# abeauvisage/uasl_motion_estimation

Hardware: AMD Instinct MI355X
Metric: frames/sec + BA iter/sec, 2000 feats x 20-keyframe window, 1/2/4/8 MI355X (higher is better)
Workload: dtype u8+f32 (MI), f64 (BA); 1 GPU; config 3: 1280x720 stereo, 2000 feats, 20-keyframe window, 11x11 MI patches; frame=KLT + MI scale LM (LM, MAX_NB_ITER 10, tolerances off) + 10 BA LM iterations, parallelism=1 independent streams (one per GPU)

## Files before the change

### uasl_motion_estimation_amd/csrc/api.hip

```cpp
#include <vector>
#include "me_internal.hpp"
#include <algorithm>
#include <cstring>
#include <rocprofiler-sdk-roctx/roctx.h>

me_range::me_range(const char* name) { roctxRangePushA(name); }
me_range::~me_range() { roctxRangePop(); }

typedef float me_f4v __attribute__((ext_vector_type(4)));
__global__ __launch_bounds__(256) void copy_f4_kernel(const me_f4v* __restrict__ a, me_f4v* __restrict__ b, size_t n) {
  const size_t stride = (size_t)gridDim.x * 256;
  for (size_t i = (size_t)blockIdx.x * 256 + threadIdx.x; i < n; i += stride)
    __builtin_nontemporal_store(__builtin_nontemporal_load(&a[i]), &b[i]);
}

static int hbm_copy_gbs(me_ctx* c, size_t bytes, int reps, double* gbs) {
  void *a = nullptr, *b = nullptr;
  ME_HIP(c, hipMalloc(&a, bytes));
  hipError_t e = hipMalloc(&b, bytes);
  if (e != hipSuccess) {
    (void)hipFree(a);
    return me_set_error(c, ME_ERR_NOMEM, "me_hbm_copy_gbs: hipMalloc(%zu) failed", bytes);
  }
  const size_t n = bytes / 16;
// ... 16 lines not shown
  if (e0) (void)hipEventDestroy(e0);
  if (e1) (void)hipEventDestroy(e1);
  (void)hipFree(a);
  (void)hipFree(b);
  if (rc == ME_OK) *gbs = 2.0 * (double)(n * 16) * reps / (ms * 1e-3) / 1e9;
  return rc;
}

int me_set_error(me_ctx* ctx, int code, const char* fmt, ...) {
  if (ctx) {
    char buf[1024];
    va_list ap;
    va_start(ap, fmt);
    vsnprintf(buf, sizeof(buf), fmt, ap);
    va_end(ap);
    ctx->err = buf;
  }
  return code;
}

int me_scratch(me_ctx* ctx, int slot, size_t bytes, void** out) {
  if ((int)ctx->slot_ptr.size() <= slot) {
    ctx->slot_ptr.resize(slot + 1, nullptr);
    ctx->slot_size.resize(slot + 1, 0);
  }
  if (bytes == 0) bytes = 16;
  if (ctx->slot_size[slot] < bytes) {
    if (ctx->slot_ptr[slot]) {
      ME_HIP(ctx, hipStreamSynchronize(ctx->stream));
      ME_HIP(ctx, hipFree(ctx->slot_ptr[slot]));
      ctx->slot_ptr[slot] = nullptr;
      ctx->slot_size[slot] = 0;
    }
    size_t sz = bytes + bytes / 4;
    void* p = nullptr;
    hipError_t e = hipMalloc(&p, sz);
    if (e != hipSuccess) return me_set_error(ctx, ME_ERR_NOMEM, "hipMalloc(%zu) failed: %s", sz, hipGetErrorString(e));
    ctx->slot_ptr[slot] = p;
    ctx->slot_size[slot] = sz;
  }
  *out = ctx->slot_ptr[slot];
  return ME_OK;
}

int me_pinned(me_ctx* ctx, size_t bytes, void** out) {
  if (ctx->pinned_size < bytes) {
    if (ctx->pinned) {
      ME_HIP(ctx, hipStreamSynchronize(ctx->stream));
      ME_HIP(ctx, hipHostFree(ctx->pinned));
    }
    ctx->pinned = nullptr;
    ctx->pinned_size = 0;
    size_t sz = bytes < 4096 ? 4096 : bytes;
    ME_HIP(ctx, hipHostMalloc(&ctx->pinned, sz, hipHostMallocDefault));
    ctx->pinned_size = sz;
  }
  *out = ctx->pinned;
  return ME_OK;
}

int me_check_launch(me_ctx* ctx, const char* what) {
  hipError_t e = hipGetLastError();
  if (e != hipSuccess) return me_set_error(ctx, ME_ERR_HIP, "launch of %s failed: %s", what, hipGetErrorString(e));
  return ME_OK;
}

static hipEvent_t pool_get(me_ctx* c) {
  if (!c->event_pool.empty()) {
    hipEvent_t e = c->event_pool.back();
    c->event_pool.pop_back();
    return e;
  }
  hipEvent_t e = nullptr;
  if (hipEventCreate(&e) != hipSuccess) return nullptr;
  return e;
}

me_ktimer::me_ktimer(me_ctx* ctx, int kernel, bool ext_launch) : c(ctx), k(kernel), ext(ext_launch) {
  if (c && (c->timing >> kernel & 1) && c->kt_seen[kernel]++ % c->timing_every == 0) {
    a = pool_get(c);
    b = pool_get(c);
    if (!a || !b) a = b = nullptr;
    if (a && !ext) hipEventRecord(a, c->stream);
  }
}
me_ktimer::~me_ktimer() {
  if (c && a && b) {
    if (!ext) hipEventRecord(b, c->stream);
    c->pending.push_back({a, b, k});
  }
}

static void drain_timers(me_ctx* c) {
  for (auto& p : c->pending) {
    hipEventSynchronize(p.b);
    float ms = 0;
    if (hipEventElapsedTime(&ms, p.a, p.b) == hipSuccess) {
      c->launches[p.kernel] += 1;
      c->total_ms[p.kernel] += ms;
    }
    c->event_pool.push_back(p.a);
    c->event_pool.push_back(p.b);
  }
  c->pending.clear();
}

extern "C" {
// ... 184 lines not shown
```

### uasl_motion_estimation_amd/csrc/ba.hip

```cpp
#include <algorithm>
#include <cmath>
#include <cstdio>
#include <cstring>
#include <mutex>
#include <numeric>
#include <vector>
#include <hip/hip_ext.h>
#include "me_internal.hpp"
#include "ba_kernels.hpp"
#include "roster.hpp"
#include "solve_diag.hpp"
#include "me_device.hpp"

using me_dev::wave_sync;

using namespace ba;

namespace {

constexpr double kDblMin = 2.2250738585072014e-308;
constexpr double kDblEps = 2.220446049250313e-16;

template <int Ctrl>
__device__ __forceinline__ double dpp_f64(double x);
// ... 176 lines not shown
  }
  for (int k = 12; k < 24; ++k) Jc[k] = 0.0;
  for (int k = 6; k < 12; ++k) Jp[k] = 0.0;
}

template <int OD>
__device__ __forceinline__ void obs_residual(const Geo& g, const Bufs& b, long o, const double* cam, const double* X,
                                             double* r, double* Jc, double* Jp) {
  if (OD == 4)
    stereo_residual(g, cam, X, b.obs + 4 * o, r, Jc, Jp);
  else
    mono_residual(g, cam, X, b.obs + 2 * o, b.cam_id[o] != 0, r, Jc, Jp);
}

__device__ __forceinline__ void huber(double s, double* rho0, double* sqrt_rho1) {
  if (s > 1.0) {
    const double rr = sqrt(s);
    *rho0 = 2.0 * rr - 1.0;
    *sqrt_rho1 = sqrt(fmax(kDblMin, 1.0 / rr));
  } else {
    *rho0 = s;
    *sqrt_rho1 = 1.0;
  }
}

template <bool SC1>
__device__ __forceinline__ double a_ld(const double* p) {
  if (!SC1) return *p;
  return __builtin_bit_cast(double, __hip_atomic_load(reinterpret_cast<const unsigned long long*>(p), ME_HO_LD,
                                                      __HIP_MEMORY_SCOPE_AGENT));
}
template <bool SC1>
__device__ __forceinline__ void a_st(double* p, double v) {
  if (!SC1) {
    *p = v;
    return;
  }
  __hip_atomic_store(reinterpret_cast<unsigned long long*>(p), __builtin_bit_cast(unsigned long long, v),
                     ME_HO_ST, __HIP_MEMORY_SCOPE_AGENT);
}
__device__ __forceinline__ void drain_and_barrier() {
  asm volatile("s_waitcnt vmcnt(0)" ::: "memory");
  __syncthreads();
}


constexpr int kPtBlock = 64;

#ifndef ME_LIN_SMALL
#define ME_LIN_SMALL 64
#endif
constexpr int kLinSmall = ME_LIN_SMALL, kLinSmallMaxObs = 64 * 512;
__host__ __device__ inline int lin_block(int no) { return no <= kLinSmallMaxObs ? kLinSmall : kBlock; }
template <int OD, int BLK>
__global__ __launch_bounds__(BLK) void linearize_kernel(Geo g, Bufs b) {
  __shared__ double lds[BLK / 64];
  const State* st = b.st;
  if (st->done || !st->need_lin) return;
  const int o = blockIdx.x * BLK + threadIdx.x;
  double cost = 0;
  if (o < g.no) {
    const int cur = st->cur;
    const int ci = b.cam_idx[o], pi = b.pt_idx[o];
    double r[4], Jc[24], Jp[12];
    obs_residual<OD>(g, b, o, b.cams[cur] + 6 * ci, b.pts[cur] + 3 * pi, r, Jc, Jp);
    const double s = r[0] * r[0] + r[1] * r[1] + r[2] * r[2] + r[3] * r[3];
    double rho0, sc;
    huber(s, &rho0, &sc);
    cost = 0.5 * rho0;
    for (int k = 0; k < 4; ++k) r[k] *= sc;
    for (int k = 0; k < 24; ++k) Jc[k] *= sc;
    for (int k = 0; k < 12; ++k) Jp[k] *= sc;
    const long slot = b.pos[o];
    double* X = b.obsx + slot * kObsxStride;
    X[0] = Jp[0] * Jp[0] + Jp[3] * Jp[3] + Jp[6] * Jp[6] + Jp[9] * Jp[9];
    X[1] = Jp[0] * Jp[1] + Jp[3] * Jp[4] + Jp[6] * Jp[7] + Jp[9] * Jp[10];
    X[2] = Jp[0] * Jp[2] + Jp[3] * Jp[5] + Jp[6] * Jp[8] + Jp[9] * Jp[11];
    X[3] = Jp[1] * Jp[1] + Jp[4] * Jp[4] + Jp[7] * Jp[7] + Jp[10] * Jp[10];
    X[4] = Jp[1] * Jp[2] + Jp[4] * Jp[5] + Jp[7] * Jp[8] + Jp[10] * Jp[11];
    X[5] = Jp[2] * Jp[2] + Jp[5] * Jp[5] + Jp[8] * Jp[8] + Jp[11] * Jp[11];
    for (int a = 0; a < 3; ++a) X[6 + a] = Jp[a] * r[0] + Jp[3 + a] * r[1] + Jp[6 + a] * r[2] + Jp[9 + a] * r[3];
    if (ci - g.nf >= 0) {
      double* W = b.Wo + 18 * slot;
      for (int a = 0; a < 6; ++a)
        for (int c = 0; c < 3; ++c)
          W[a * 3 + c] = Jc[a] * Jp[c] + Jc[6 + a] * Jp[3 + c] + Jc[12 + a] * Jp[6 + c] + Jc[18 + a] * Jp[9 + c];
    }
  }
  double v[1] = {cost};
  double out[1];
  block_sum<1>(v, out, lds);
  if (threadIdx.x == 0) b.part[R_COST * g.pstride + blockIdx.x] = out[0];
}

__device__ __forceinline__ bool last_arrival_wt(unsigned* cnt, unsigned expected) {
  __shared__ int slast;
  __syncthreads();
  if (threadIdx.x == 0) {
    asm volatile("s_waitcnt vmcnt(0)" ::: "memory");
    const unsigned k = __hip_atomic_fetch_add(cnt, 1u, ME_HO_RMW, __HIP_MEMORY_SCOPE_AGENT);
    slast = k == expected - 1;
    if (slast) __hip_atomic_store(cnt, 0u, __ATOMIC_RELAXED, __HIP_MEMORY_SCOPE_AGENT);
  }
  __syncthreads();
  return slast != 0;
}

__device__ void cam_reduce_body(const Geo& g, const Bufs& b, int sharded, const double* cpart, double* colnorm,
                                double* gc_raw, double* Uraw, int ci, int first, int count) {
  __shared__ double tot[27];
  __shared__ double csl[6];
  const State* st = b.st;
  const int u = threadIdx.x;
  if (u < 27) {
    double sum = 0.0;
    for (int k = 0; k < count; ++k) sum += a_ld<true>(&cpart[27 * ((long)first + k) + u]);
    tot[u] = sum;
    if (u < 21) Uraw[21 * (long)ci + u] = sum;
    else gc_raw[6 * ci + u - 21] = sum;
  }
  __syncthreads();
  if (u < 6) {
    const int d = u * 6 - u * (u - 1) / 2;
    colnorm[6 * ci + u] = tot[d];
    if (!sharded) {
      double* cs = b.csc + 6 * ci;
      if (!st->scaled) cs[u] = g.jacobi ? 1.0 / (1.0 + sqrt(tot[d])) : 1.0;
      csl[u] = cs[u];
    }
  }
  if (sharded) return;
  __syncthreads();
  if (u < 21) {
    int a = 0, r = u;
    while (r >= 6 - a) {
      r -= 6 - a;
      ++a;
    }
    const int c = a + r;
    const double x = tot[u] * csl[a] * csl[c];
    double* U = b.U + 36 * (long)ci;
// ... 49 lines not shown
    huber(s2, &rho0, &sc);
    for (int kk = 0; kk < 4; ++kk) r[kk] *= sc;
    for (int kk = 0; kk < 24; ++kk) Jc[kk] *= sc;
    int u = 0;
    for (int a = 0; a < 6; ++a)
      for (int c = a; c < 6; ++c, ++u)
        v[u] += Jc[a] * Jc[c] + Jc[6 + a] * Jc[6 + c] + Jc[12 + a] * Jc[12 + c] + Jc[18 + a] * Jc[18 + c];
    for (int a = 0; a < 6; ++a) v[21 + a] += Jc[a] * r[0] + Jc[6 + a] * r[1] + Jc[12 + a] * r[2] + Jc[18 + a] * r[3];
  }
  CAM_T(1);
#pragma unroll
  for (int u = 0; u < 27; ++u) {
    double x = v[u];
    x += dpp_f64<kDppQuadSwap1>(x);
    x += dpp_f64<kDppQuadSwap2>(x);
    x += dpp_f64<kDppRowHalfMirror>(x);
    x += dpp_f64<kDppRowMirror>(x);
    v[u] = x;
  }
  if ((threadIdx.x & 15) == 0)
#pragma unroll
    for (int u = 0; u < 27; ++u) rows[(threadIdx.x >> 4) * 27 + u] = v[u];
  __syncthreads();
  CAM_T(2);
  if (threadIdx.x < 27) {
    double sum = 0.0;
#pragma unroll
    for (int r = 0; r < kBlock / 16; ++r) sum += rows[r * 27 + threadIdx.x];
    a_st<true>(&cpart[27 * (long)un + threadIdx.x], sum);
  }
  const bool last = last_arrival_wt(b.cnt + ci, (unsigned)ue.w);
  CAM_T(3);
  if (!last) return;
  cam_reduce_body(g, b, sharded, cpart, colnorm, gc_raw, Uraw, ci, ufirst, ue.w);
  CAM_T(4);
#ifdef ME_CAM_TS
  if (un == g_cam_ts_unit && threadIdx.x == 0) atomicAdd(&g_cam_ts[5], 1ull);
#endif
}

__global__ __launch_bounds__(kBlock) void cam_assemble_kernel(Geo g, Bufs b, double* cpart, int sharded,
                                                              double* colnorm, double* gc_raw, double* Uraw) {
  if (g.od == 4)
    cam_assemble_body<4>(g, b, cpart, sharded, colnorm, gc_raw, Uraw, blockIdx.x);
  else
    cam_assemble_body<2>(g, b, cpart, sharded, colnorm, gc_raw, Uraw, blockIdx.x);
}

struct CamArgs {
  double *cpart, *colnorm, *gc_raw, *Uraw;
  int on;
  int ncam;
};

__global__ void xch_flags_kernel(Geo g, Bufs b, double* colnorm) {
  colnorm[g.n6] = b.st->bad_input ? 1.0 : 0.0;
  colnorm[g.n6 + 1] = b.st->infeasible ? 1.0 : 0.0;
}

__global__ void cam_finish_kernel(Geo g, Bufs b, const double* colnorm, const double* gc_raw, const double* Uraw,
                                  int first) {
  State* st = b.st;
  if (first) {
    const bool bad = colnorm[g.n6] != 0.0, infeasible = colnorm[g.n6 + 1] != 0.0;
    __syncthreads();
    if (bad || infeasible) {
      if (blockIdx.x == 0 && threadIdx.x == 0) {
        st->bad_input = bad;
        st->infeasible = infeasible;
        st->done = 1;
        st->termination = 2;
      }
      return;
    }
  }
  if (st->done || !st->need_lin) return;
  const int ci = blockIdx.x * blockDim.x + threadIdx.x;
  if (ci >= g.m) return;
  double* cs = b.csc + 6 * ci;
  if (!st->scaled)
    for (int a = 0; a < 6; ++a) cs[a] = g.jacobi ? 1.0 / (1.0 + sqrt(colnorm[6 * ci + a])) : 1.0;
  const double* Ur = Uraw + 21 * (long)ci;
  double* U = b.U + 36 * (long)ci;
  int u = 0;
  for (int a = 0; a < 6; ++a)
    for (int c = a; c < 6; ++c, ++u) {
      const double x = Ur[u] * cs[a] * cs[c];
      U[a * 6 + c] = x;
      U[c * 6 + a] = x;
    }
  for (int a = 0; a < 6; ++a) b.gcs[6 * ci + a] = gc_raw[6 * ci + a] * cs[a];
}

__device__ __forceinline__ bool chol3(const double* A, double* L) {
  double d0 = A[0];
  if (!(d0 > 0)) return false;
  d0 = sqrt(d0);
  const double l10 = A[3] / d0, l20 = A[6] / d0;
  double d1 = A[4] - l10 * l10;
  if (!(d1 > 0)) return false;
  d1 = sqrt(d1);
  const double l21 = (A[7] - l20 * l10) / d1;
  double d2 = A[8] - l20 * l20 - l21 * l21;
  if (!(d2 > 0)) return false;
  d2 = sqrt(d2);
  L[0] = d0; L[1] = 0; L[2] = 0;
// ... 2171 lines not shown
  int run = wsum[wv] + x - s;
  for (long i = beg; i < end; ++i) {
    const int v = b.phist[i];
    b.phist[i] = run;
    run += v;
  }
  __syncthreads();
  for (int j = t; j < g.np; j += kScanBlock) {
    const int key = b.pkey[j];
    const int pos = b.phist[(long)key * g.nblkp + j / kBlock] + b.prank[j];
    b.order[pos] = j;
    const int r = pos / g.rlen;
    if (pos == r * g.rlen) rA[r] = key / g.T;
    atomicMax(&rB[r], key % g.T);
  }
  __syncthreads();
  for (int r = t; r < g.nruns; r += kScanBlock) {
    const int B = max(rA[r], rB[r]);
    rB[r] = B;
    b.rband[2 * r] = rA[r];
    b.rband[2 * r + 1] = B;
  }
  __syncthreads();
  for (int p = t; p < g.npairs; p += kScanBlock) {
    int I = 0, rem = p;
    while (rem >= g.T - I) {
      rem -= g.T - I;
      ++I;
    }
    const int J = I + rem;
    int cnt = 0;
    for (int r = 0; r < g.nruns; ++r) {
      const int A = rA[r], B = rB[r];
      const int nb = B - A + 1, ns = nb + (B < g.T - 1 ? 1 : 0);
      const int ka = (I >= A && I <= B) ? I - A : (I == g.T - 1 ? nb : -1);
      const int kb = (J >= A && J <= B) ? J - A : (J == g.T - 1 ? nb : -1);
      if (ka < 0 || kb < 0) continue;
      b.tl[(long)p * g.nruns + cnt++] = r * g.npairs + ka * ns - ka * (ka - 1) / 2 + (kb - ka);
    }
    b.tcnt[p] = cnt;
    for (int q = cnt; q < g.nruns; ++q) b.tl[(long)p * g.nruns + q] = -1;
  }
}

__global__ __launch_bounds__(kBlock) void output_kernel(Geo g, Bufs b, double* cams_dst, double* pts_dst) {
  const int cur = b.st->cur;
  const long gid = (long)blockIdx.x * kBlock + threadIdx.x;
  constexpr int kStateWords = (int)(sizeof(State) / 8);
  if (gid < kStateWords) b.out[gid] = ((const double*)b.st)[gid];
  if (gid < 6 * (long)g.nc) cams_dst[gid] = b.cams[cur][gid];
  if (gid < 3 * (long)g.np) pts_dst[gid] = b.pts[cur][gid];
}

struct Plan {
  me_ctx* c = nullptr;
  Geo g;
  unsigned asm_gen = 0;
  Bufs b;
  Opts o;
  double* colnorm = nullptr;
  double* gc_raw = nullptr;
  double* Uraw = nullptr;
  double* cpart = nullptr;
  double* host = nullptr;
  State* hstate[2] = {nullptr, nullptr};
  bool dev = false;
  bool copy_out = false;
  bool reserve_only = false;
  size_t solve_lds = 0;
  size_t schur_lds = 0;
  int use_lds = 0;
  int solve_flags = 0;
  int n_enq = 0;
  bool no_fused_asm = false;
  bool full_S = false;
  int solve_cap = 0;
  me_comm* comm = nullptr;
  bool xmax_separate = false;
};

inline long rup(long x, long m) { return (x + m - 1) / m * m; }
int blocks(long n, int bs) { return (int)std::max(1L, (n + bs - 1) / bs); }

void schur_geometry(int npairs, int np, int Rpad, Geo& g) {
  const bool wide = schur_lds_bytes(kSchurPtsWide, Rpad) <= kSchurLdsCap;
  const bool split_wide = wide && npairs <= 40 && np <= 256 * kSchurPts;
  g.spts = wide ? kSchurPtsWide : npairs > 100 ? kSchurPtsSmall : kSchurPts;
  g.nsub = (int)std::max(1L, ((long)np + g.spts - 1) / g.spts);
  g.rsub = (int)std::max(1L, ((long)g.nsub + 255) / 256);
  g.rlen = g.spts * g.rsub;
  g.nruns = (int)std::max(1L, ((long)np + g.rlen - 1) / g.rlen);
  const int nt = split_wide ? 2 : npairs > 100 ? kSchurNtMax : std::min(kSchurNtMax, 4);
  g.stpw = 8 * std::min((npairs + 7) / 8, nt);
  g.sgrp = (npairs + g.stpw - 1) / g.stpw;
  g.ksplit = (g.sgrp > 1 ? (int)rup((long)g.nruns, 8) : g.nruns) * g.sgrp;
  g.sorted = npairs > 40 ? 1 : 0;
}

void ba_geometry(Geo& g, int n_cams, int fixed_frames, int n_pts) {
  g.nc = n_cams;
  g.np = n_pts;
  g.nf = std::min(std::max(fixed_frames, 0), n_cams);
  g.m = g.nc - g.nf;
  g.n6 = 6 * g.m;
  g.Rpad = (int)rup(g.n6 + 1, 16);
  g.T = g.Rpad / 16;
  g.Ts = (g.n6 + 1 + 15) / 16;
  g.npairs = g.T * (g.T + 1) / 2;
  schur_geometry(g.npairs, g.np, g.Rpad, g);
}

constexpr size_t kSolveLdsCap = 150 * 1024;
inline int solve_form(int Ts) {
  if (8 * (solve_small_doubles(Ts) + solve_a_doubles(Ts)) <= kSolveLdsCap) return 0;
  return Ts >= kSolveMwMinTs ? 2 : 1;
}

extern "C" int me_debug_ba_geometry(int n_cams, int fixed_frames, int n_pts, int* out) {
  if (n_cams <= 0 || n_pts < 0 || !out) return ME_ERR_INVALID;
  Geo g;
  ba_geometry(g, n_cams, fixed_frames, n_pts);
  const int v[10] = {g.spts, g.nsub, g.rsub, g.rlen, g.nruns, g.stpw, g.sgrp, g.ksplit, g.sorted, solve_form(g.Ts)};
  std::memcpy(out, v, sizeof v);
  return ME_OK;
}

int ba_drain(me_ctx* c);

int plan_build(me_ctx* c, const me_ba_problem* p, const me_ba_options* opt, Plan& P, int slot_base,
               int async = -1, me_comm* comm = nullptr) {
  if (async < 0) ME_TRY(ba_drain(c));
  ME_CHECK(c, p->n_cams > 0 && p->n_pts >= 0 && p->n_obs >= 0, "BA: bad sizes");
  ME_CHECK(c, p->n_cams <= kMaxScanCams, "BA: at most %d cameras per window", kMaxScanCams);
  ME_CHECK(c, p->obs_dim == 0 || p->obs_dim == 2 || p->obs_dim == 4, "BA: obs_dim must be 2 or 4 (Observation<M>)");
  const bool mono = p->obs_dim == 2;
  ME_CHECK(c, p->feat_var > 0 && (mono || p->baseline != 0.0), "BA: wrong calibration parameters (BundleAdjuster.h:147)");
  ME_CHECK(c, !mono || p->cam_id || p->n_obs == 0, "BA: obs_dim 2 needs cam_id (Observation::camID)");
  const double baseline = mono && p->baseline == 0 ? 0.5 : p->baseline;
  ME_CHECK(c, p->mem == ME_HOST || p->mem == ME_DEVICE, "BA: bad memory kind");
  if (p->mem == ME_HOST) {
    for (int i = 0; i < p->n_obs; ++i) {
      ME_CHECK(c, p->cam_idx[i] >= 0 && p->cam_idx[i] < p->n_cams && p->pt_idx[i] >= 0 && p->pt_idx[i] < p->n_pts,
               "BA: observation %d indexes outside the window", i);
    }
  }
  P.c = c;
  int hook = c->dbg_solve_flags;
  if ((hook & kFlagFailEveryOther) && (c->dbg_solve_count++ & 1)) hook |= kFlagSolveFail;
  P.no_fused_asm = (hook & kFlagSeparateAsm) != 0;
  P.solve_flags = hook & (kFlagAsmTimeout | kFlagSolveFail | kFlagRosterNow);
  Geo& g = P.g;
  ba_geometry(g, p->n_cams, p->fixed_frames, p->n_pts);
  g.no = p->n_obs;
  g.od = mono ? 2 : 4;
  P.comm = comm;
  P.xmax_separate = comm && comm->world == 0;
  g.xslots = comm && comm->world > 0 ? comm->world : 1;
  g.xrank = comm && comm->world > 0 ? comm->rank : 0;
  ME_CHECK(c, g.nruns <= kMaxRuns, "BA: %d Schur runs exceed %d", g.nruns, kMaxRuns);
  g.nblkp = blocks(std::max(g.np, 1), kBlock);
  ME_CHECK(c, g.npairs <= 8 * 24, "BA: %d variable cameras exceed the Schur tile budget", g.m);
  g.nblk_obs = (int)std::max(1L, rup(std::max(g.no, 1), kBlock) / kBlock);
  g.nblk_lin = (int)std::max(1L, rup(std::max(g.no, 1), lin_block(g.no)) / lin_block(g.no));
  g.nblk_pts = (int)std::max(1L, rup(std::max(g.np, 1), kPtBlock) / kPtBlock);
  g.jacobi = opt->jacobi_scaling ? 1 : 0;
  g.ncu = (int)(rup(std::max(g.no, 1), kBlock) / kBlock) + g.m;
  g.nblk_step = (int)std::max(1L, rup(std::max(g.np, 1), kStepPts) / kStepPts);
  g.pstride = std::max({g.nblk_obs, g.nblk_lin, g.nblk_pts, g.nblk_step, g.ksplit});
  std::memcpy(g.K0, p->K0, sizeof(g.K0));
  std::memcpy(g.K1, p->K1, sizeof(g.K1));
  g.baseline = baseline;
  g.sinv = 1.0 / std::sqrt(p->feat_var);
  const double Zmax = p->K0[0] * baseline / 0.1;
  const double Zmin = p->K0[0] * baseline / (2 * p->K0[2]);
  g.hi[0] = Zmax / p->K0[0] * p->K0[2];
  g.hi[1] = Zmax / p->K0[4] * p->K0[5];
  g.hi[2] = Zmax;
  g.lo[0] = -Zmax / p->K0[0] * p->K0[2];
  g.lo[1] = -Zmax / p->K0[4] * p->K0[5];
  g.lo[2] = Zmin;
// ... 12 lines not shown
  const bool dev = p->mem == ME_DEVICE;
  const long nb = g.pstride;
  Bufs& b = P.b;
  std::vector<std::pair<size_t, void**>> items;
  auto add = [&](size_t bytes, void* dst) { items.push_back({rup((long)std::max<size_t>(bytes, 8), 256), (void**)dst}); };
  add(8 * 6 * (size_t)g.nc, &b.cams[0]);
  add(8 * 3 * (size_t)g.np, &b.pts[0]);
  add(8 * g.od * (size_t)g.no, &b.obs);
  add(4 * (size_t)g.no, &b.cam_idx);
  add(4 * (size_t)g.no, &b.pt_idx);
  add(mono ? 4 * (size_t)g.no : 0, &b.cam_id);
  const size_t n_inputs = items.size();
  add(8 * 6 * (size_t)g.nc, &b.cams[1]);
  add(8 * 3 * (size_t)g.np, &b.pts[1]);
  add(4 * (size_t)(g.np + 1), &b.p_off);
  add(4 * (size_t)g.no, &b.p_obs);
  add(4 * (size_t)g.no, &b.pos);
  add(4 * (size_t)g.no, &b.p_cam);
  add(4 * (size_t)(g.m + 1), &b.c_off);
  add(4 * (size_t)g.no, &b.c_obs);
  add(4 * (size_t)g.no, &b.tmp_obs);
  add(4 * (size_t)g.no, &b.cpos);
  add(8 * kObsxStride * (size_t)g.no, &b.obsx);
  add((size_t)g.no, &b.dup);
  add(8 * solve_a_doubles(g.Ts), &b.Abuf);
  add(8 * 18 * (size_t)g.no, &b.Wo);
  add(8 * (size_t)g.n6, &b.csc);
  add(8 * 3 * (size_t)g.np, &b.psc);
  add(8 * 36 * (size_t)g.m, &b.U);
  add(8 * (size_t)g.n6, &b.gcs);
  add(8 * 9 * (size_t)g.np, &b.V);
  add(8 * 3 * (size_t)g.np, &b.gps);
  add(8 * 9 * (size_t)g.np, &b.Lp);
  add(8 * 3 * (size_t)g.np, &b.zp);
  add(8 * 256 * (size_t)g.nruns * g.npairs, &b.Spart);
  add(4 * (size_t)std::max(g.np, 1), &b.order);
  add(4 * (size_t)std::max(g.np, 1), &b.pkey);
  add(4 * (size_t)std::max(g.np, 1), &b.prank);
  add(4 * (size_t)g.T * g.T * g.nblkp, &b.phist);
  add(8 * (size_t)g.nruns, &b.rband);
  add(4 * (size_t)g.npairs * g.nruns, &b.tl);
  add(4 * (size_t)g.npairs, &b.tcnt);
  add(8 * (size_t)g.n6 * g.n6 + 8 * (size_t)(2 * g.n6 + 2), &b.S);
  add(8 * (size_t)g.n6, &b.yc);
  add(8 * 3 * (size_t)g.np, &b.dp);
  add(8 * R_COUNT * (size_t)nb, &b.part);
  add(8 * (R_COUNT + 2), &b.scal);
  add(sizeof(State), &b.st);
  add(8 * (size_t)(g.n6 + 2), &P.colnorm);
  add(8 * (size_t)g.n6, &P.gc_raw);
  add(8 * 21 * (size_t)std::max(g.m, 1), &P.Uraw);
  add(8 * 27 * (size_t)g.ncu, &P.cpart);
  add(4 * (size_t)kCuStride * (size_t)rup(g.ncu, 8), &b.cunit);
  add(4 * (size_t)(g.m + 1 + 3 + 2), &b.cnt);
  add(4 * (size_t)blocks((long)g.npairs * 256, kSolveBlock / kSaGroups), &b.asm_claim);
  const size_t work_bytes = 4 * (2 * (size_t)g.np + (size_t)g.nblk_obs * g.nc + 4);
  add(work_bytes, &b.work);
  const size_t out_doubles = sizeof(State) / 8 + 6 * (size_t)g.nc + 3 * (size_t)g.np;
  add(8 * out_doubles, &b.out);
  b.xch = nullptr;
  if (comm) add(8 * (size_t)xo_total(g), &b.xch);
  size_t total = 0, input_span = 0;
  for (size_t k = 0; k < items.size(); ++k) {
    total += items[k].first;
    if (k < n_inputs) input_span += items[k].first;
  }
  void* arena;
  ME_TRY(me_scratch(c, SLOT_COUNT + slot_base, total, &arena));
  char* ptr = (char*)arena;
  for (auto& it : items) {
    *it.second = ptr;
    ptr += it.first;
  }
  b.ssync = b.cnt + g.m + 1;
  b.roster = b.cnt + g.m + 4;
  b.bvec = b.S + (size_t)g.n6 * g.n6;
  b.diagU = b.bvec + g.n6;
  void* hp;
  const size_t stage = rup((long)std::max(8 * out_doubles, dev ? (size_t)0 : input_span), 64);
  const size_t hbytes = stage + 2 * rup(sizeof(State), 64);
  if (async >= 0) {
    if (c->ba_pinned_size[async] < hbytes) {
      if (c->ba_pinned[async]) ME_HIP(c, hipHostFree(c->ba_pinned[async]));
      c->ba_pinned[async] = nullptr;
      c->ba_pinned_size[async] = 0;
      ME_HIP(c, hipHostMalloc(&c->ba_pinned[async], std::max(hbytes, (size_t)4096), hipHostMallocDefault));
      c->ba_pinned_size[async] = std::max(hbytes, (size_t)4096);
    }
    hp = c->ba_pinned[async];
  } else {
    ME_TRY(me_pinned(c, hbytes, &hp));
  }
  P.host = (double*)hp;
  if (P.reserve_only) return ME_OK;
  P.hstate[0] = (State*)((char*)hp + stage);
  P.hstate[1] = (State*)((char*)hp + stage + rup(sizeof(State), 64));
  P.dev = dev;
  hipStream_t s = c->stream;
  if (!dev) {
    char* h = (char*)hp;
    const void* src[6] = {p->cams, p->pts, p->obs, p->cam_idx, p->pt_idx, p->cam_id};
    const size_t len[6] = {8 * 6 * (size_t)g.nc, 8 * 3 * (size_t)g.np, 8 * g.od * (size_t)g.no, 4 * (size_t)g.no,
                           4 * (size_t)g.no, mono ? 4 * (size_t)g.no : 0};
    size_t off = 0;
    for (int k = 0; k < 6; ++k) {
      if (len[k]) std::memcpy(h + off, src[k], len[k]);
      off += items[k].first;
    }
    ME_HIP(c, hipMemcpyAsync(b.cams[0], hp, input_span, hipMemcpyHostToDevice, s));
  } else {
    b.obs = p->obs;
    b.cam_idx = p->cam_idx;
    b.pt_idx = p->pt_idx;
    if (mono) b.cam_id = p->cam_id;
  }
  ME_HIP(c, hipMemsetAsync(b.cnt, 0, (size_t)((char*)b.work - (char*)b.cnt) + work_bytes, s));
  P.asm_gen = 0;
  const double* cams_in = dev ? p->cams : b.cams[0];
  const double* pts_in = dev ? p->pts : b.pts[0];
  const long nthr = std::max({(long)g.nblk_obs * kBlock, (long)g.np, 6L * g.nc, 3L * g.np});
  hipLaunchKernelGGL(plan_count_kernel, dim3(blocks(nthr, kBlock)), dim3(kBlock), 4 * (size_t)g.nc, s, g, b, cams_in,
                     pts_in);
  hipLaunchKernelGGL(plan_scan_kernel, dim3(1), dim3(kScanBlock), 0, s, g, b, o);
  hipLaunchKernelGGL(plan_scatter_kernel, dim3(g.nblk_obs), dim3(kBlock), 0, s, g, b);
  hipLaunchKernelGGL(plan_segsort_kernel, dim3(blocks(std::max(g.np, 1), kSortBlock / 64)), dim3(kSortBlock), 0, s, g,
                     b);
  if (g.sorted) {
    hipLaunchKernelGGL(plan_band_kernel, dim3(g.nblkp), dim3(kBlock), 0, s, g, b);
    hipLaunchKernelGGL(plan_order_kernel, dim3(1), dim3(kScanBlock), 0, s, g, b);
  }
  ME_TRY(me_check_launch(c, "BA plan"));
  P.use_lds = solve_form(g.Ts) == 0 ? 1 : 0;
  P.solve_lds = 8 * (solve_small_doubles(g.Ts) + (P.use_lds ? solve_a_doubles(g.Ts) : 0));
  ME_CHECK(c, P.solve_lds <= kSolveLdsCap, "BA: %d variable cameras exceed the camera-solve workspace", g.m);
  P.schur_lds = schur_lds_bytes(g.spts, g.Rpad);
  ME_CHECK(c, P.schur_lds <= kSchurLdsCap, "BA: %d variable cameras exceed the Schur workspace", g.m);
  if (!c->ba_lds_attr) {
    for (const void* k : {(const void*)cam_solve_kernel<0>, (const void*)cam_solve_kernel<1>, (const void*)cam_solve_kernel<2>})
      ME_HIP(c, hipFuncSetAttribute(k, hipFuncAttributeMaxDynamicSharedMemorySize, (int)kSolveLdsCap));
#define ME_SCHUR_K(N)                                                                                   \
  (const void*)pt_schur_kernel<N, 512, kSchurPts>, (const void*)pt_schur_kernel<N, 512, kSchurPtsWide>, \
      (const void*)pt_schur_kernel<N, 512, kSchurPtsSmall>
    for (const void* k : {ME_SCHUR_K(2), ME_SCHUR_K(3), ME_SCHUR_K(4), ME_SCHUR_K(5)})
#undef ME_SCHUR_K
      ME_HIP(c, hipFuncSetAttribute(k, hipFuncAttributeMaxDynamicSharedMemorySize, (int)kSchurLdsCap));
    c->ba_lds_attr = 1;
  }
  if (!P.use_lds) {
    int per_cu = 0;
    ME_HIP(c, hipOccupancyMaxActiveBlocksPerMultiprocessor(&per_cu, cam_solve_kernel<2>, kSolveBlock, P.solve_lds));
    P.solve_cap = std::max(0, per_cu) * (c->cu_active > 0 ? c->cu_active : c->num_cu);
    if (P.comm && g.Ts >= kSolveMwMinTs) {
      double* d = P.b.scal;
      const double v = -(double)P.solve_cap;
      ME_HIP(c, hipMemcpyAsync(d, &v, 8, hipMemcpyHostToDevice, c->stream));
      ME_TRY(me_comm_allreduce_impl(P.comm, d, 1, ME_COMM_MAX));
      double r = 0.0;
      ME_HIP(c, hipMemcpyAsync(&r, d, 8, hipMemcpyDeviceToHost, c->stream));
      ME_HIP(c, hipStreamSynchronize(c->stream));
      P.solve_cap = (int)-r;
    }
  }
  return ME_OK;
}



#define ME_XCH(ptr, n, op) ME_TRY(me_comm_allreduce_impl(P.comm, (ptr), (long)(n), (op)))

int enqueue_linearize(Plan& P) {
  me_ctx* c = P.c;
  const Geo& g = P.g;
  hipStream_t s = c->stream;
  const bool sh = P.comm != nullptr;
  {
    me_ktimer t(c, ME_KT_BA_LINEARIZE);
    const bool small = lin_block(g.no) == kLinSmall;
    if (g.od == 4 && small)
      hipLaunchKernelGGL((linearize_kernel<4, kLinSmall>), dim3(g.nblk_lin), dim3(kLinSmall), 0, s, g, P.b);
    else if (g.od == 4)
      hipLaunchKernelGGL((linearize_kernel<4, kBlock>), dim3(g.nblk_lin), dim3(kBlock), 0, s, g, P.b);
    else if (small)
      hipLaunchKernelGGL((linearize_kernel<2, kLinSmall>), dim3(g.nblk_lin), dim3(kLinSmall), 0, s, g, P.b);
    else
      hipLaunchKernelGGL((linearize_kernel<2, kBlock>), dim3(g.nblk_lin), dim3(kBlock), 0, s, g, P.b);
  }
  const bool first = P.n_enq == 0;
  const bool fused = !first && g.m > 0;
  ++P.n_enq;
  CamArgs ca{P.cpart, P.colnorm, P.gc_raw, P.Uraw, fused ? 1 : 0, fused ? (g.ncu + 7) / 8 * 8 : 0};
  if (g.m > 0 && !fused)
    hipLaunchKernelGGL(cam_assemble_kernel, dim3(g.ncu), dim3(kBlock), 0, s, g, P.b, P.cpart, sh ? 1 : 0,
                       P.colnorm, P.gc_raw, P.Uraw);
  if (sh && !fused) {
    if (first) {
      hipLaunchKernelGGL(xch_flags_kernel, dim3(1), dim3(1), 0, s, g, P.b, P.colnorm);
      ME_XCH(P.colnorm, g.n6 + 2, ME_COMM_SUM);
    }
    hipLaunchKernelGGL(cam_finish_kernel, dim3(blocks(std::max(g.m, 1), 64)), dim3(64), 0, s, g, P.b,
                       (const double*)P.colnorm, (const double*)P.gc_raw, (const double*)P.Uraw, first ? 1 : 0);
  }
  {
    me_ktimer t(c, ME_KT_BA_SCHUR, true);
    const int pw8 = g.stpw / 8;
    const dim3 grd(g.ksplit + ca.ncam);
#define ME_SCHUR(N)                                                                                          \
  do {                                                                                                       \
    if (g.spts == kSchurPtsWide)                                                                             \
      hipExtLaunchKernelGGL((pt_schur_kernel<N, 512, kSchurPtsWide>), grd, dim3(512), P.schur_lds, s, t.a, t.b, 0, g, \
                            P.b, P.o, ca);                                                                   \
    else if (g.spts == kSchurPtsSmall)                                                                       \
      hipExtLaunchKernelGGL((pt_schur_kernel<N, 512, kSchurPtsSmall>), grd, dim3(512), P.schur_lds, s, t.a, t.b, 0, g, \
                            P.b, P.o, ca);                                                                   \
    else                                                                                                     \
      hipExtLaunchKernelGGL((pt_schur_kernel<N, 512, kSchurPts>), grd, dim3(512), P.schur_lds, s, t.a, t.b, 0, g, P.b, \
                            P.o, ca);                                                                        \
  } while (0)
    static_assert(kSchurNtMax >= 3 && kSchurNtMax <= 5, "instantiated tile counts");
    if (pw8 <= 2) ME_SCHUR(2);
    else if (pw8 <= 3) ME_SCHUR(3);
    else if (pw8 <= 4) ME_SCHUR(4);
    else ME_SCHUR(5);
#undef ME_SCHUR
  }
  if (sh) {
    hipLaunchKernelGGL(s_assemble_kernel, dim3(blocks((long)g.npairs * 256, kSaElems) + 1), dim3(kBlock), 0, s, g,
                       P.b, P.o, (const double*)P.gc_raw, 0, (int)SA_PACK);
    if (P.xmax_separate) {
      ME_XCH(P.b.xch, xo_gmax(g), ME_COMM_SUM);
      ME_XCH(P.b.xch + xo_gmax(g), 1, ME_COMM_MAX);
    } else {
      ME_XCH(P.b.xch, xo_total(g), ME_COMM_SUM);
    }
  }
  return me_check_launch(c, "BA linearize");
}

int enqueue_assemble(Plan& P, bool img = false) {
  me_ctx* c = P.c;
  const Geo& g = P.g;
  const int mode = P.comm ? SA_UNPACK : SA_SUM;
  if (g.m > 0)
    hipLaunchKernelGGL(s_assemble_kernel, dim3(blocks((long)g.npairs * 256, kSaElems) + 1), dim3(kBlock), 0,
                       c->stream, g, P.b, P.o, (const double*)P.gc_raw, P.full_S ? 1 : 0, mode,
                       img && !P.full_S ? P.b.Abuf : nullptr);
  else
    hipLaunchKernelGGL(lin_finalize_kernel, dim3(1), dim3(kFinBlock), 0, c->stream, g, P.b, P.o,
                       (const double*)P.gc_raw);
  return me_check_launch(c, "BA assemble");
}

int enqueue_iteration(Plan& P, bool last = false) {
  me_ctx* c = P.c;
  const Geo& g = P.g;
  hipStream_t s = c->stream;
  const bool sh = P.comm != nullptr;
  ME_TRY(enqueue_linearize(P));
  const int np0 = (g.Ts - 1) * g.Ts / 2;
  int nwk = solve_form(g.Ts) == 2 ? std::min(64, std::max(1, (np0 + kSolveBlock / 64 - 1) / (kSolveBlock / 64))) : 0;
  nwk = std::max(0, std::min(nwk, P.solve_cap - 1));
  const bool fuse = g.m > 0 && !P.full_S && !last && nwk == 0 && !P.no_fused_asm;
  const int nasm = fuse ? blocks((long)g.npairs * 256, kSolveBlock / kSaGroups) : 0;
  const bool img = !fuse && !last && g.m > 0 && !P.full_S && ME_SOLVE_IMG;
  if (!fuse) ME_TRY(enqueue_assemble(P, img));
  if (last) return me_check_launch(c, "BA iteration");
  if (g.m == 0) ME_HIP(c, hipMemsetAsync(P.b.scal + R_COUNT, 0, 8, s));
  {
    me_ktimer t(c, ME_KT_BA_SOLVE);
    const double* gc = P.gc_raw;
    const int sk = P.solve_flags | (img ? kFlagImg : 0);
    const unsigned gen = nasm > 0 ? ++P.asm_gen : 0u;
    if (P.use_lds)
      hipLaunchKernelGGL(cam_solve_kernel<0>, dim3(1 + nasm), dim3(kSolveBlock), P.solve_lds, s, g, P.b, P.o, sk, 0,
                         nasm, gc, gen);
    else if (nwk > 0)
#ifdef ME_COOP_LAUNCH
    {
      int skv = sk, nwv = nwk, z = 0;
      unsigned gv = gen;
      void* args[] = {(void*)&g, (void*)&P.b, (void*)&P.o, &skv, &nwv, &z, (void*)&gc, &gv};
      ME_HIP(c, hipLaunchCooperativeKernel((const void*)cam_solve_kernel<2>, dim3(1 + nwk), dim3(kSolveBlock), args,
                                           (unsigned)P.solve_lds, s));
    }
#else
      hipLaunchKernelGGL(cam_solve_kernel<2>, dim3(1 + nwk), dim3(kSolveBlock), P.solve_lds, s, g, P.b, P.o, sk, nwk,
                         0, gc, gen);
#endif
    else
      hipLaunchKernelGGL(cam_solve_kernel<1>, dim3(1 + nasm), dim3(kSolveBlock), P.solve_lds, s, g, P.b, P.o, sk, 0,
                         nasm, gc, gen);
  }
  {
    me_ktimer t(c, ME_KT_BA_STEP);
    if (g.od == 4)
      hipLaunchKernelGGL(pt_step_kernel<4>, dim3(g.nblk_step + 1), dim3(kStepBlock), 0, s, g, P.b, P.o, sh ? 0 : 1);
    else
      hipLaunchKernelGGL(pt_step_kernel<2>, dim3(g.nblk_step + 1), dim3(kStepBlock), 0, s, g, P.b, P.o, sh ? 0 : 1);
  }
  if (sh) {
    ME_XCH(P.b.scal + R_MODEL, 5, ME_COMM_SUM);
    hipLaunchKernelGGL(decide_kernel, dim3(1), dim3(64), 0, s, g, P.b, P.o);
  }
  return me_check_launch(c, "BA iteration");
}

int enqueue_output(Plan& P, me_ba_problem* p) {
  me_ctx* c = P.c;
  const Geo& g = P.g;
  constexpr size_t nst = sizeof(State) / 8;
  double* cams_dst = P.dev ? p->cams : P.b.out + nst;
  double* pts_dst = P.dev ? p->pts : P.b.out + nst + 6 * (size_t)g.nc;
  const long n = std::max({(long)nst, 6L * g.nc, 3L * g.np});
  hipLaunchKernelGGL(output_kernel, dim3(blocks(n, kBlock)), dim3(kBlock), 0, c->stream, g, P.b, cams_dst, pts_dst);
  ME_TRY(me_check_launch(c, "BA output"));
  const size_t bytes = 8 * (P.dev ? nst : nst + 6 * (size_t)g.nc + 3 * (size_t)g.np);
  ME_HIP(c, hipMemcpyAsync(P.host, P.b.out, bytes, hipMemcpyDeviceToHost, c->stream));
  if (P.dev && P.copy_out) {
    ME_HIP(c, hipMemcpyAsync(P.host + nst, p->cams, 8 * 6 * (size_t)g.nc, hipMemcpyDeviceToHost, c->stream));
    if (g.np)
      ME_HIP(c, hipMemcpyAsync(P.host + nst + 6 * (size_t)g.nc, p->pts, 8 * 3 * (size_t)g.np, hipMemcpyDeviceToHost,
                               c->stream));
  }
  return ME_OK;
}

int finish(Plan& P, me_ba_problem* p, me_ba_summary* sum, bool output_queued = false, hipEvent_t done = nullptr) {
  me_ctx* c = P.c;
  const Geo& g = P.g;
  constexpr size_t nst = sizeof(State) / 8;
  static_assert(sizeof(State) % 8 == 0, "State is read back as doubles");
  if (!output_queued) ME_TRY(enqueue_output(P, p));
  if (done) ME_HIP(c, hipEventSynchronize(done));
  else ME_HIP(c, hipStreamSynchronize(c->stream));
  State st;
  std::memcpy(&st, P.host, sizeof(State));
  std::memcpy(P.c->dbg, st.stamps, sizeof(st.stamps));
  if (!P.dev) {
    std::memcpy(p->cams, P.host + nst, 8 * 6 * (size_t)g.nc);
    if (g.np) std::memcpy(p->pts, P.host + nst + 6 * (size_t)g.nc, 8 * 3 * (size_t)g.np);
  }
  if (st.bad_input) return me_set_error(c, ME_ERR_INVALID, "BA: an observation indexes outside the window");
  if (st.spin_err)
    return me_set_error(c, ME_ERR_STATE,
                        "BA: a cross-workgroup hand-off of the camera solve timed out (workgroups not co-resident: "
                        "CU mask or concurrent persistent kernels; wait sites 0x%x: 1 worker roster, 2 worker step "
                        "poll, 4 fused assemblers, 8 LDS step flags, 16 workers' count, 32 backward flags, 0 the "
                        "step exchange)",
                        (unsigned)st.pad[0]);
  if (sum) {
    sum->termination = st.termination;
    sum->iterations = st.iterations;
    sum->successful_steps = st.successful;
    sum->initial_cost = st.initial_cost;
    sum->final_cost = st.x_cost;
    sum->status = st.termination == 2 ? 3 : 2;
    if (st.infeasible) {
      sum->iterations = 0;
      sum->successful_steps = 0;
      sum->initial_cost = sum->final_cost = NAN;
    }
  }
  return ME_OK;
}

int solve_impl(me_ctx* c, me_ba_problem* p, const me_ba_options* opt, me_comm* comm, me_ba_summary* sum) {
  me_range range_("me_ba_solve");
  if (!c || !p || !opt) return ME_ERR_INVALID;
  ME_HIP(c, hipSetDevice(c->device));
  Plan P;
  ME_TRY(plan_build(c, p, opt, P, 0, -1, comm));
  const int chunk = 4;
  int it = 0;
  auto enqueue_chunk = [&](int slot) -> int {
    for (int k = 0; k < chunk && it <= opt->max_num_iterations; ++k, ++it)
      ME_TRY(enqueue_iteration(P, it == opt->max_num_iterations));
    ME_HIP(c, hipMemcpyAsync(P.hstate[slot], P.b.st, sizeof(State), hipMemcpyDeviceToHost, c->stream));
    ME_HIP(c, hipEventRecord(c->poll_ev[slot], c->stream));
    return ME_OK;
  };
  bool out_q = false;
  ME_TRY(enqueue_chunk(0));
  if (it > opt->max_num_iterations) {
    ME_TRY(enqueue_output(P, p));
    out_q = true;
  }
  for (int cur = 0;; cur ^= 1) {
    const bool more = it <= opt->max_num_iterations;
    if (more) {
      ME_TRY(enqueue_chunk(cur ^ 1));
      if (it > opt->max_num_iterations) {
        ME_TRY(enqueue_output(P, p));
        out_q = true;
      }
    }
    ME_HIP(c, hipEventSynchronize(c->poll_ev[cur]));
    if (P.hstate[cur]->done || !more) break;
  }
  return finish(P, p, sum, out_q);
}

struct AsyncSolve {
  Plan P;
  me_ba_problem prob;
  hipEvent_t ev = nullptr;
  int set = 0;
  bool completed = false;
  int rc = ME_OK;
  me_ba_summary sum{};
};
constexpr int kBaQueue = 2;
struct AsyncQueue {
  AsyncSolve* q[kBaQueue] = {nullptr, nullptr};
  int n = 0;
  AsyncSolve* last = nullptr;
  int last_set = 1;
  std::mutex mu;
};

int ba_complete_one(me_ctx* c, AsyncSolve* A) {
  if (A->completed) return ME_OK;
  A->rc = finish(A->P, &A->prob, &A->sum, true, A->ev);
  A->completed = true;
  return ME_OK;
}

void ba_async_free(me_ctx* c) {
  auto* Q = (AsyncQueue*)c->ba_async;
  if (!Q) return;
  for (int i = 0; i < Q->n; ++i) {
    AsyncSolve* A = Q->q[i];
    if (!A->completed) hipEventSynchronize(A->ev);
    hipEventDestroy(A->ev);
    delete A;
  }
  delete Q->last;
  delete Q;
  c->ba_async = nullptr;
  c->ba_async_free = nullptr;
}

AsyncQueue* ba_queue(me_ctx* c) {
  if (!c->ba_async) {
    c->ba_async = new AsyncQueue;
    c->ba_async_free = ba_async_free;
  }
  return (AsyncQueue*)c->ba_async;
}

int ba_drain(me_ctx* c) {
  auto* Q = (AsyncQueue*)c->ba_async;
  if (!Q) return ME_OK;
  for (int i = 0; i < Q->n; ++i) ME_TRY(ba_complete_one(c, Q->q[i]));
  return ME_OK;
}

AsyncSolve* ba_chain_source(AsyncQueue* Q) {
  std::lock_guard<std::mutex> lk(Q->mu);
  return Q->n ? Q->q[Q->n - 1] : Q->last;
}

}

static int solve_async_impl(me_ctx* c, me_ba_problem* p, const me_ba_options* opt, bool copy_out) {
// ... 501 lines not shown
```

### uasl_motion_estimation_amd/csrc/me_internal.hpp

```cpp
#pragma once
#include <hip/hip_runtime.h>
#include <cstdarg>
#include <cstdio>
#include <string>
#include <vector>
#include "../../include/me_hip.h"

struct me_timer_pair {
  hipEvent_t a, b;
  int kernel;
};

enum : int {
  kFlagAsmTimeout = 512,
  kFlagSolveFail = 1024,
  kFlagFailEveryOther = 2048,
  kFlagImg = 4096,
  kFlagRosterNow = 8192,
  kFlagSeparateAsm = 16384,
  kFlagMiLane = 32768,
  kHookMask = kFlagAsmTimeout | kFlagSolveFail | kFlagFailEveryOther | kFlagRosterNow | kFlagSeparateAsm | kFlagMiLane,
};

struct me_ctx {
  int device = 0;
  int num_cu = 256;
  int cu_active = 0;
  hipStream_t own_stream = nullptr;
  hipStream_t stream = nullptr;
  std::string err;
  std::vector<void*> slot_ptr;
  std::vector<size_t> slot_size;
  void* pinned = nullptr;
  size_t pinned_size = 0;
  int timing = 0;
  std::vector<me_timer_pair> pending;
  std::vector<hipEvent_t> event_pool;
  long launches[ME_KT_COUNT] = {0};
  double total_ms[ME_KT_COUNT] = {0};
  long kt_seen[ME_KT_COUNT] = {0};
  int timing_every = 1;
  hipEvent_t poll_ev[2] = {nullptr, nullptr};
  int32_t rand_st[31] = {0};
  int rand_f = 3, rand_r = 0;
  bool rand_init = false;
  long long dbg[16] = {0};
  int dbg_solve_flags = 0;
  unsigned dbg_solve_count = 0;
  void* ba_async = nullptr;
  void (*ba_async_free)(me_ctx*) = nullptr;
  void* ba_pinned[2] = {nullptr, nullptr};
  size_t ba_pinned_size[2] = {0, 0};
  int ba_lds_attr = 0;
  void* scale_mirror = nullptr;
  int scale_gen = 0;
  int scale_lm_cap = -1;
  long scale_counters[4] = {0, 0, 0, 0};
  float* mi_table[256] = {nullptr};
};

struct me_comm {
  me_ctx* ctx = nullptr;
  int world = 1, rank = 0;
  void* nccl = nullptr;
  me_allreduce_fn ar = nullptr;
  void* user = nullptr;
  double xch_us[2] = {0.0, 0.0};
};
int me_comm_allreduce_impl(me_comm* m, double* buf, long n, int op);

int me_mi_table(me_ctx* ctx, int npx, const float** out);

int me_set_error(me_ctx* ctx, int code, const char* fmt, ...);

#define ME_HIP(ctx, call)                                                                    \
  do {                                                                                       \
    hipError_t e_ = (call);                                                                  \
    if (e_ != hipSuccess)                                                                    \
      return me_set_error((ctx), ME_ERR_HIP, "%s failed: %s (%s:%d)", #call, hipGetErrorString(e_), \
                          __FILE__, __LINE__);                                               \
  } while (0)

#define ME_CHECK(ctx, cond, ...)                                     \
  do {                                                               \
    if (!(cond)) return me_set_error((ctx), ME_ERR_INVALID, __VA_ARGS__); \
  } while (0)

#define ME_TRY(expr)            \
  do {                          \
    int rc_ = (expr);           \
    if (rc_ != ME_OK) return rc_; \
  } while (0)

int me_scratch(me_ctx* ctx, int slot, size_t bytes, void** out);
int me_pinned(me_ctx* ctx, size_t bytes, void** out);
int me_check_launch(me_ctx* ctx, const char* what);

struct me_range {
  explicit me_range(const char* name);
  ~me_range();
};

struct me_ktimer {
  me_ctx* c;
  int k;
// ... 13 lines not shown
```

Measured before the change: 1362 frames/s.

## Merge first linearize with camera assembly and fold BA close into one kernel

The first BA iteration now launches a single kernel that runs camera assembly blocks alongside linearize blocks, removing one launch. The final iteration skips the redundant assemble and runs one close kernel that finalizes, copies state, cams and points out, and re-zeroes the counter scratch. The next solve can then skip its memset when the same stream reuses that scratch set. Pinned buffers switch to coherent host allocation. Together these cut launches and host-device round trips per solve, at the cost of extra clean-flag bookkeeping and some correctness risk if the scratch is reused across streams.

```diff
diff --git a/uasl_motion_estimation_amd/csrc/api.hip b/uasl_motion_estimation_amd/csrc/api.hip
--- a/uasl_motion_estimation_amd/csrc/api.hip
+++ b/uasl_motion_estimation_amd/csrc/api.hip
@@ -92,7 +92,7 @@
     ctx->pinned = nullptr;
     ctx->pinned_size = 0;
     size_t sz = bytes < 4096 ? 4096 : bytes;
-    ME_HIP(ctx, hipHostMalloc(&ctx->pinned, sz, hipHostMallocDefault));
+    ME_HIP(ctx, hipHostMalloc(&ctx->pinned, sz, hipHostMallocCoherent));
     ctx->pinned_size = sz;
   }
   *out = ctx->pinned;
diff --git a/uasl_motion_estimation_amd/csrc/ba.hip b/uasl_motion_estimation_amd/csrc/ba.hip
--- a/uasl_motion_estimation_amd/csrc/ba.hip
+++ b/uasl_motion_estimation_amd/csrc/ba.hip
@@ -252,12 +252,8 @@
 #endif
 constexpr int kLinSmall = ME_LIN_SMALL, kLinSmallMaxObs = 64 * 512;
 __host__ __device__ inline int lin_block(int no) { return no <= kLinSmallMaxObs ? kLinSmall : kBlock; }
-template <int OD, int BLK>
-__global__ __launch_bounds__(BLK) void linearize_kernel(Geo g, Bufs b) {
-  __shared__ double lds[BLK / 64];
-  const State* st = b.st;
-  if (st->done || !st->need_lin) return;
-  const int o = blockIdx.x * BLK + threadIdx.x;
+template <int OD>
+__device__ __forceinline__ double lin_obs_body(const Geo& g, const Bufs& b, const State* st, int o) {
   double cost = 0;
   if (o < g.no) {
     const int cur = st->cur;
@@ -287,6 +283,15 @@
           W[a * 3 + c] = Jc[a] * Jp[c] + Jc[6 + a] * Jp[3 + c] + Jc[12 + a] * Jp[6 + c] + Jc[18 + a] * Jp[9 + c];
     }
   }
+  return cost;
+}
+
+template <int OD, int BLK>
+__global__ __launch_bounds__(BLK) void linearize_kernel(Geo g, Bufs b) {
+  __shared__ double lds[BLK / 64];
+  const State* st = b.st;
+  if (st->done || !st->need_lin) return;
+  const double cost = lin_obs_body<OD>(g, b, st, blockIdx.x * BLK + threadIdx.x);
   double v[1] = {cost};
   double out[1];
   block_sum<1>(v, out, lds);
@@ -442,6 +447,33 @@
   int on;
   int ncam;
 };
+
+#ifndef ME_FIRST_MERGED
+#define ME_FIRST_MERGED 1
+#endif
+template <int OD, int PB>
+__global__ __launch_bounds__(kBlock) void first_linearize_kernel(Geo g, Bufs b, CamArgs ca) {
+  static_assert(PB == 64 || PB == kBlock, "a partial per wave or per workgroup");
+  if ((int)blockIdx.x < ca.ncam) {
+    cam_assemble_body<OD>(g, b, ca.cpart, 0, ca.colnorm, ca.gc_raw, ca.Uraw, blockIdx.x);
+    return;
+  }
+  __shared__ double lds[kBlock / 64];
+  const State* st = b.st;
+  if (st->done || !st->need_lin) return;
+  const int lb = (int)blockIdx.x - ca.ncam;
+  const double cost = lin_obs_body<OD>(g, b, st, lb * kBlock + threadIdx.x);
+  if (PB == 64) {
+    const double t = wave_total(cost);
+    const int pb = lb * (kBlock / 64) + (threadIdx.x >> 6);
+    if ((threadIdx.x & 63) == 0 && pb < g.nblk_lin) b.part[R_COST * g.pstride + pb] = 0.0 + t;
+  } else {
+    double v[1] = {cost};
+    double out[1];
+    block_sum<1>(v, out, lds);
+    if (threadIdx.x == 0) b.part[R_COST * g.pstride + lb] = out[0];
+  }
+}
 
 __global__ void xch_flags_kernel(Geo g, Bufs b, double* colnorm) {
   colnorm[g.n6] = b.st->bad_input ? 1.0 : 0.0;
@@ -2719,6 +2751,35 @@
   if (gid < 3 * (long)g.np) pts_dst[gid] = b.pts[cur][gid];
 }
 
+__global__ __launch_bounds__(kBlock) void close_kernel(Geo g, Bufs b, Opts o, const double* gc_raw, double* cams_dev,
+                                                       double* pts_dev, double* host_state, double* cams_host,
+                                                       double* pts_host, uint4* zero, long nzero) {
+  static_assert(kBlock == kFinBlock, "the finalize block runs with the copy block size");
+  constexpr int kStateWords = (int)(sizeof(State) / 8);
+  static_assert(kStateWords <= kBlock, "State is stored by one workgroup");
+  for (long i = (long)blockIdx.x * kBlock + threadIdx.x; i < nzero; i += (long)gridDim.x * kBlock)
+    zero[i] = make_uint4(0u, 0u, 0u, 0u);
+  if (blockIdx.x == 0) {
+    __shared__ double lds[16];
+    lin_finalize_body(g, b, o, gc_raw, lds);
+    __syncthreads();
+    if (threadIdx.x < kStateWords) host_state[threadIdx.x] = ((const double*)b.st)[threadIdx.x];
+    return;
+  }
+  const int cur = b.st->cur;
+  const long gid = (long)(blockIdx.x - 1) * kBlock + threadIdx.x;
+  if (gid < 6 * (long)g.nc) {
+    const double v = b.cams[cur][gid];
+    if (cams_dev) cams_dev[gid] = v;
+    if (cams_host) cams_host[gid] = v;
+  }
+  if (gid < 3 * (long)g.np) {
+    const double v = b.pts[cur][gid];
+    if (pts_dev) pts_dev[gid] = v;
+    if (pts_host) pts_host[gid] = v;
+  }
+}
+
 struct Plan {
   me_ctx* c = nullptr;
   Geo g;
@@ -2734,6 +2795,9 @@
   bool dev = false;
   bool copy_out = false;
   bool reserve_only = false;
+  int set = 0;
+  void* zero = nullptr;
+  size_t zero_bytes = 0;
   size_t solve_lds = 0;
   size_t schur_lds = 0;
   int use_lds = 0;
@@ -2793,6 +2857,11 @@
 }
 
 int ba_drain(me_ctx* c);
+#ifndef ME_ONCE_CLOSE
+#define ME_ONCE_CLOSE 1
+#endif
+constexpr int kBaSets = 2;
+static_assert(kBaSets == sizeof(me_ctx::ba_clean) / sizeof(int), "one clean flag per scratch set");
 
 int plan_build(me_ctx* c, const me_ba_problem* p, const me_ba_options* opt, Plan& P, int slot_base,
                int async = -1, me_comm* comm = nullptr) {
@@ -2911,10 +2980,6 @@
   add(8 * 21 * (size_t)std::max(g.m, 1), &P.Uraw);
   add(8 * 27 * (size_t)g.ncu, &P.cpart);
   add(4 * (size_t)kCuStride * (size_t)rup(g.ncu, 8), &b.cunit);
-  add(4 * (size_t)(g.m + 1 + 3 + 2), &b.cnt);
-  add(4 * (size_t)blocks((long)g.npairs * 256, kSolveBlock / kSaGroups), &b.asm_claim);
-  const size_t work_bytes = 4 * (2 * (size_t)g.np + (size_t)g.nblk_obs * g.nc + 4);
-  add(work_bytes, &b.work);
   const size_t out_doubles = sizeof(State) / 8 + 6 * (size_t)g.nc + 3 * (size_t)g.np;
   add(8 * out_doubles, &b.out);
   b.xch = nullptr;
@@ -2930,6 +2995,25 @@
   for (auto& it : items) {
     *it.second = ptr;
     ptr += it.first;
+  }
+  {
+    const size_t zb[3] = {
+        (size_t)rup(4 * (long)(g.m + 1 + 3 + 2), 256),
+        (size_t)rup(4 * (long)blocks((long)g.npairs * 256, kSolveBlock / kSaGroups), 256),
+        (size_t)rup(4 * (2 * (long)g.np + (long)g.nblk_obs * g.nc + 4), 256)};
+    const int zslot = SLOT_COUNT + kBaSets + slot_base;
+    const size_t had = (int)c->slot_size.size() > zslot ? c->slot_size[zslot] : 0;
+    ME_TRY(me_scratch(c, zslot, zb[0] + zb[1] + zb[2], &P.zero));
+    if (c->slot_size[zslot] != had) {
+      ME_HIP(c, hipMemsetAsync(P.zero, 0, c->slot_size[zslot], c->stream));
+      c->ba_clean[slot_base] = 1;
+      c->ba_clean_stream[slot_base] = c->stream;
+    }
+    P.set = slot_base;
+    P.zero_bytes = zb[0] + zb[1] + zb[2];
+    b.cnt = (unsigned*)P.zero;
+    b.asm_claim = (unsigned*)((char*)P.zero + zb[0]);
+    b.work = (int*)((char*)P.zero + zb[0] + zb[1]);
   }
   b.ssync = b.cnt + g.m + 1;
   b.roster = b.cnt + g.m + 4;
@@ -2943,7 +3027,7 @@
       if (c->ba_pinned[async]) ME_HIP(c, hipHostFree(c->ba_pinned[async]));
       c->ba_pinned[async] = nullptr;
       c->ba_pinned_size[async] = 0;
-      ME_HIP(c, hipHostMalloc(&c->ba_pinned[async], std::max(hbytes, (size_t)4096), hipHostMallocDefault));
+      ME_HIP(c, hipHostMalloc(&c->ba_pinned[async], std::max(hbytes, (size_t)4096), hipHostMallocCoherent));
       c->ba_pinned_size[async] = std::max(hbytes, (size_t)4096);
     }
     hp = c->ba_pinned[async];
@@ -2973,7 +3057,10 @@
     b.pt_idx = p->pt_idx;
     if (mono) b.cam_id = p->cam_id;
   }
-  ME_HIP(c, hipMemsetAsync(b.cnt, 0, (size_t)((char*)b.work - (char*)b.cnt) + work_bytes, s));
+  const bool clean = ME_ONCE_CLOSE && c->ba_clean[P.set] && c->ba_clean_stream[P.set] == s;
+  c->ba_clean[P.set] = 0;
+  if (!clean)
+    ME_HIP(c, hipMemsetAsync(P.zero, 0, ME_ONCE_CLOSE ? c->slot_size[SLOT_COUNT + kBaSets + P.set] : P.zero_bytes, s));
   P.asm_gen = 0;
   const double* cams_in = dev ? p->cams : b.cams[0];
   const double* pts_in = dev ? p->pts : b.pts[0];
@@ -3032,9 +3119,23 @@
   const Geo& g = P.g;
   hipStream_t s = c->stream;
   const bool sh = P.comm != nullptr;
-  {
+  const bool first = P.n_enq == 0;
+  const bool small = lin_block(g.no) == kLinSmall;
+  const bool merged = ME_FIRST_MERGED && first && !sh && g.m > 0 && (!small || kLinSmall == 64);
+  if (merged) {
     me_ktimer t(c, ME_KT_BA_LINEARIZE);
-    const bool small = lin_block(g.no) == kLinSmall;
+    const CamArgs ca{P.cpart, P.colnorm, P.gc_raw, P.Uraw, 1, (g.ncu + 7) / 8 * 8};
+    const dim3 grd(ca.ncam + blocks(g.no, kBlock));
+    if (g.od == 4 && small)
+      hipLaunchKernelGGL((first_linearize_kernel<4, 64>), grd, dim3(kBlock), 0, s, g, P.b, ca);
+    else if (g.od == 4)
+      hipLaunchKernelGGL((first_linearize_kernel<4, kBlock>), grd, dim3(kBlock), 0, s, g, P.b, ca);
+    else if (small)
+      hipLaunchKernelGGL((first_linearize_kernel<2, 64>), grd, dim3(kBlock), 0, s, g, P.b, ca);
+    else
+      hipLaunchKernelGGL((first_linearize_kernel<2, kBlock>), grd, dim3(kBlock), 0, s, g, P.b, ca);
+  } else {
+    me_ktimer t(c, ME_KT_BA_LINEARIZE);
     if (g.od == 4 && small)
       hipLaunchKernelGGL((linearize_kernel<4, kLinSmall>), dim3(g.nblk_lin), dim3(kLinSmall), 0, s, g, P.b);
     else if (g.od == 4)
@@ -3044,11 +3145,10 @@
     else
       hipLaunchKernelGGL((linearize_kernel<2, kBlock>), dim3(g.nblk_lin), dim3(kBlock), 0, s, g, P.b);
   }
-  const bool first = P.n_enq == 0;
   const bool fused = !first && g.m > 0;
   ++P.n_enq;
   CamArgs ca{P.cpart, P.colnorm, P.gc_raw, P.Uraw, fused ? 1 : 0, fused ? (g.ncu + 7) / 8 * 8 : 0};
-  if (g.m > 0 && !fused)
+  if (g.m > 0 && !fused && !merged)
     hipLaunchKernelGGL(cam_assemble_kernel, dim3(g.ncu), dim3(kBlock), 0, s, g, P.b, P.cpart, sh ? 1 : 0,
                        P.colnorm, P.gc_raw, P.Uraw);
   if (sh && !fused) {
@@ -3109,6 +3209,8 @@
   return me_check_launch(c, "BA assemble");
 }
 
+inline bool closes_in_one(const Plan& P) { return ME_ONCE_CLOSE && !P.comm && !P.full_S; }
+
 int enqueue_iteration(Plan& P, bool last = false) {
   me_ctx* c = P.c;
   const Geo& g = P.g;
@@ -3121,7 +3223,7 @@
   const bool fuse = g.m > 0 && !P.full_S && !last && nwk == 0 && !P.no_fused_asm;
   const int nasm = fuse ? blocks((long)g.npairs * 256, kSolveBlock / kSaGroups) : 0;
   const bool img = !fuse && !last && g.m > 0 && !P.full_S && ME_SOLVE_IMG;
-  if (!fuse) ME_TRY(enqueue_assemble(P, img));
+  if (!fuse && !(last && closes_in_one(P))) ME_TRY(enqueue_assemble(P, img));
   if (last) return me_check_launch(c, "BA iteration");
   if (g.m == 0) ME_HIP(c, hipMemsetAsync(P.b.scal + R_COUNT, 0, 8, s));
   {
@@ -3167,6 +3269,18 @@
   me_ctx* c = P.c;
   const Geo& g = P.g;
   constexpr size_t nst = sizeof(State) / 8;
+  if (closes_in_one(P)) {
+    const bool stage = !P.dev || P.copy_out;
+    const long n = std::max(6L * g.nc, 3L * g.np);
+    hipLaunchKernelGGL(close_kernel, dim3(1 + blocks(n, kBlock)), dim3(kBlock), 0, c->stream, g, P.b, P.o,
+                       (const double*)P.gc_raw, P.dev ? p->cams : nullptr, P.dev ? p->pts : nullptr, P.host,
+                       stage ? P.host + nst : nullptr, stage ? P.host + nst + 6 * (size_t)g.nc : nullptr,
+                       (uint4*)P.zero, (long)(P.zero_bytes / 16));
+    ME_TRY(me_check_launch(c, "BA close"));
+    c->ba_clean[P.set] = 1;
+    c->ba_clean_stream[P.set] = c->stream;
+    return ME_OK;
+  }
   double* cams_dst = P.dev ? p->cams : P.b.out + nst;
   double* pts_dst = P.dev ? p->pts : P.b.out + nst + 6 * (size_t)g.nc;
   const long n = std::max({(long)nst, 6L * g.nc, 3L * g.np});
@@ -3267,7 +3381,7 @@
   int rc = ME_OK;
   me_ba_summary sum{};
 };
-constexpr int kBaQueue = 2;
+constexpr int kBaQueue = kBaSets;
 struct AsyncQueue {
   AsyncSolve* q[kBaQueue] = {nullptr, nullptr};
   int n = 0;
diff --git a/uasl_motion_estimation_amd/csrc/me_internal.hpp b/uasl_motion_estimation_amd/csrc/me_internal.hpp
--- a/uasl_motion_estimation_amd/csrc/me_internal.hpp
+++ b/uasl_motion_estimation_amd/csrc/me_internal.hpp
@@ -51,6 +51,8 @@
   void (*ba_async_free)(me_ctx*) = nullptr;
   void* ba_pinned[2] = {nullptr, nullptr};
   size_t ba_pinned_size[2] = {0, 0};
+  int ba_clean[2] = {0, 0};
+  hipStream_t ba_clean_stream[2] = {nullptr, nullptr};
   int ba_lds_attr = 0;
   void* scale_mirror = nullptr;
   int scale_gen = 0;
```

Measured after the change: 1372 frames/s, median of 6. No clear change (+0.7%).
